# kav-institute/SemanticLiDARUnc

Hardware: AMD Instinct MI355X
Metric: range-image scans/sec (64x2048, T=8 MC) (higher is better)
Workload: dtype f16 (fp16 activations/weights, fp32 accumulate + epilogue, fp32 logits); 1 GPU; SalsaNext MC-dropout T=8 + entropy/MI map + IoU/ECE accumulation, 8 scans of 64x2048x5 per step per GPU (BASELINE configs[2] shape); T=8, parallelism=scan-sharded x1, mc_schedule=every pass fully recomputed

## Files before the change

semanticlidarunc_amd/csrc/conv_tail_h8.hip:

```cpp
#include "h8_common.h"

namespace {

struct TailArgs {
  const uint4 *a1, *a2;
  const uint4 *w2, *w1;
  const float *biasA, *bnA_a, *bnA_b, *biasB, *bnB_a, *bnB_b;
  float slopeA, slopeB;
  const uint2* resid;
  const uint4* sc_x;
  const uint4* sc_w;
  const float* sc_bias;
  float slopeS;
  uint2* out;
  int N, H, W, G;
  int tiles_x, tiles_y;
#ifdef SLU_H8_AB
  int dbg;
#endif
};

template <int MB, int WM, int WN, int RPW, bool W3RES>
__global__ __launch_bounds__(64 * WM * WN, 2) void tail_h8_kernel(const TailArgs a) {
  constexpr int NWAVE = WM * WN, T = 4, PAD = 1, DIL = 2;
// ... 441 lines not shown
              }
              const half8 bf = __builtin_bit_cast(half8, make_uint4(u[0], u[1], u[2], u[3]));
#pragma unroll
              for (int io = 0; io < MB; ++io) acco[io][b] = __builtin_amdgcn_mfma_f32_32x32x16_f16(wf[io], bf, acco[io][b], 0, 0, 0);
            }
          }
      }
    };
    h8_static_for(position, std::make_integer_sequence<int, NKS>{});
    first = false;

    if constexpr (HASRES) {
      asm volatile("s_waitcnt vmcnt(%8)"
                   : "+v"(res[0][0][0]), "+v"(res[0][0][1]), "+v"(res[(1 / NB) % MB][1 % NB][0]), "+v"(res[(1 / NB) % MB][1 % NB][1]),
                     "+v"(res[(2 / NB) % MB][2 % NB][0]), "+v"(res[(2 / NB) % MB][2 % NB][1]), "+v"(res[(3 / NB) % MB][3 % NB][0]), "+v"(res[(3 / NB) % MB][3 % NB][1])
                   : "n"(RESWAIT));
    }
    if constexpr (RES == 2) {
      static_assert(NKX * NB == 4, "the wait below names its registers");
      asm volatile("s_waitcnt vmcnt(%4)" : "+v"(xs[0][0]), "+v"(xs[0][NB - 1]), "+v"(xs[NKX - 1][0]), "+v"(xs[NKX - 1][NB - 1]) : "n"(RESWAIT));
    }
#pragma unroll
    for (int i = 0; i < MB; ++i)
#pragma unroll
      for (int b = 0; b < NB; ++b) {
        const int gy = cur.y0 + wn * RPW + (b >> 1), gx = cur.x0 + (b & 1) * 32 + jj;
        const bool ok = gy < a.H && gx < a.W;
        const size_t idx0 = ok ? ((size_t)cur.n * a.G + i * 4 + hh) * HW + (size_t)gy * a.W + gx : 0;
        f32x16 sacc;
        if constexpr (RES == 2) {
          sacc = f32x16{};
#pragma unroll
          for (int k = 0; k < NKX; ++k)
            sacc = __builtin_amdgcn_mfma_f32_32x32x16_f16(__builtin_bit_cast(half8, s_ws[(i * NKX + k) * 64 + lane]), __builtin_bit_cast(half8, xs[k][b]), sacc, 0, 0, 0);
        }
#pragma unroll
        for (int pr = 0; pr < 2; ++pr) {
          uint4 rw = make_uint4(0u, 0u, 0u, 0u);
          if constexpr (HASRES) rw = h8_swap16(res[i][b][pr].x, res[i][b][pr].y, res[i][b][pr].z, res[i][b][pr].w);
          unsigned hw[4];
#pragma unroll
          for (int q2 = 0; q2 < 2; ++q2) {
            const int q = 2 * pr + q2;
            const int c4 = (i * 32 + 8 * q) / 4;
            H8Quad t = h8_epilogue(acco[i][b], q, se4(3 * C / 4 + c4), se4(4 * C / 4 + c4), se4(5 * C / 4 + c4), slB);
            if constexpr (HASRES) h8_add_resid(t, q2 ? make_uint2(rw.z, rw.w) : make_uint2(rw.x, rw.y));
            if constexpr (RES == 2) {
              const H8Quad u = h8_bias_leaky(sacc, q, se4(6 * C / 4 + c4), slS);
              t.t0 += round_f16(u.t0);
              t.t1 += round_f16(u.t1);
            }
            hw[2 * q2] = pack2(t.t0);
            hw[2 * q2 + 1] = pack2(t.t1);
          }
          const uint4 rec = h8_swap16(hw[0], hw[1], hw[2], hw[3]);
          *(ok ? reinterpret_cast<uint4*>(a.out) + idx0 + (size_t)(2 * pr) * HW : &h8_trash_rec) = rec;
        }
      }
    asm volatile("" ::: "memory");
    cur = nxt;
    has_next = tile + 2 * t_step < t_end;
    if (has_next) nxt = decode(tile + 2 * t_step);
  }
  asm volatile("s_waitcnt vmcnt(0)" ::: "memory");
}

template <int MB, int RPW, int D, int RES>
int launch_tail2(TailArgs& a, const SluEmit& e) {
  constexpr int TH = 8 * RPW, C = 32 * MB, NKS = 2 * MB;
  constexpr size_t nblk_b = (size_t)(2 * (TH + 2) * 66 + 63) / 64;
  constexpr size_t lds = ((size_t)MB * NKS * 4 * 64 + (size_t)MB * 3 * NKS * 64 + (RES == 2 ? (size_t)MB * 2 * 64 : 0) + (size_t)D * nblk_b * 64 + 64) * 16;
  static_assert(lds + 7 * C * 4 <= 160 * 1024, "ring does not fit in LDS");
  a.tiles_x = (a.W + 63) / 64;
  a.tiles_y = (a.H + TH - 1) / TH;
  const long long nt = (long long)a.tiles_x * a.tiles_y * a.N;
  if (nt <= 0 || nt > 0x7fffffffLL) return SLU_EUNSUPPORTED;
  long long gx = 256;
  if (gx > nt) gx = nt;
  if (e.name) return slu_emit_name(e, "tail2_h8_kernel<%d, %d, %d, %d>", MB, RPW, D, RES);
  static SluLdsGrant grant;
  return slu_launch_lds(tail2_h8_kernel<MB, RPW, D, RES>, dim3((unsigned)gx), dim3(512), lds, e.st, grant, a);
}

template <int MB, int WM, int WN, int RPW, bool W3RES>
int launch_tail(TailArgs& a, const SluEmit& e) {
  constexpr int TH = WN * RPW, MBLK = MB * WM, C = 32 * MBLK, NKS = 2 * MBLK;
  constexpr size_t nb_alloc = (size_t)((2 * (TH + 2) * 66 + 63) / 64) * 64;
  constexpr size_t lds = (size_t)6 * C * 4 + 2 * nb_alloc * 16 + (size_t)2 * MBLK * 5 * 64 * 16 + (W3RES ? (size_t)MBLK * NKS * 64 * 16 : 0) +
                         (size_t)(C / 8) * TH * 64 * 16;
  static_assert(lds <= 160 * 1024, "tile does not fit in LDS");
  a.tiles_x = (a.W + 63) / 64;
  a.tiles_y = (a.H + TH - 1) / TH;
  const long long nt = (long long)a.tiles_x * a.tiles_y * a.N;
  if (nt <= 0 || nt > 0x7fffffffLL) return SLU_EUNSUPPORTED;
  long long gx = 256;
  if (gx > nt) gx = nt;
  if (e.name) return slu_emit_name(e, "tail_h8_kernel<%d, %d, %d, %d, %s>", MB, WM, WN, RPW, slu_tf(W3RES));
  static SluLdsGrant grant;
  return slu_launch_lds(tail_h8_kernel<MB, WM, WN, RPW, W3RES>, dim3((unsigned)gx), dim3(64 * WM * WN), lds, e.st, grant, a);
}

}

extern "C" int slu_conv_tail_h8_shortcut_supported(int C, int sc_cin) { return C == 64 && sc_cin == 32 ? 1 : 0; }

extern "C" int slu_conv_tail_h8_supported(int C, int H, int W) { return (C == 32 || C == 64 || C == 128) && H > 0 && W > 0 ? 1 : 0; }

static int conv_tail_dispatch(const slu_conv_tail_h8_desc* d, const SluEmit& e) {
  if (!d || !d->a1 || !d->a2 || !d->w2x2 || !d->w1x1 || !d->out || d->N <= 0 || d->H <= 0 || d->W <= 0) return SLU_EINVAL;
  if (((uintptr_t)d->a1 | (uintptr_t)d->a2 | (uintptr_t)d->out | (uintptr_t)d->resid | (uintptr_t)d->w2x2 | (uintptr_t)d->w1x1) & 15) return SLU_EINVAL;
  if ((d->bnA_a == nullptr) != (d->bnA_b == nullptr) || (d->bnB_a == nullptr) != (d->bnB_b == nullptr)) return SLU_EINVAL;
  if (!slu_conv_tail_h8_supported(d->C, d->H, d->W)) return SLU_EUNSUPPORTED;
  if (d->hasactA && !(d->slopeA >= 0.0f && d->slopeA <= 1.0f)) return SLU_EINVAL;
  if (d->hasactB && !(d->slopeB >= 0.0f && d->slopeB <= 1.0f)) return SLU_EINVAL;
  TailArgs a{};
  a.a1 = reinterpret_cast<const uint4*>(d->a1);
  a.a2 = reinterpret_cast<const uint4*>(d->a2);
  a.w2 = reinterpret_cast<const uint4*>(d->w2x2);
  a.w1 = reinterpret_cast<const uint4*>(d->w1x1);
  a.biasA = d->biasA; a.bnA_a = d->bnA_a; a.bnA_b = d->bnA_b;
  a.biasB = d->biasB; a.bnB_a = d->bnB_a; a.bnB_b = d->bnB_b;
  a.slopeA = d->hasactA ? d->slopeA : 1.0f;
  a.slopeB = d->hasactB ? d->slopeB : 1.0f;
  a.resid = reinterpret_cast<const uint2*>(d->resid);
  a.out = reinterpret_cast<uint2*>(d->out);
  a.N = d->N; a.H = d->H; a.W = d->W; a.G = d->C / 8;
#ifdef SLU_H8_AB
  static const int dbg = slu_env_int("SLU_TAIL_DBG", 0);
  a.dbg = dbg;
#endif
  static const bool v1 = slu_env_int("SLU_TAIL_V1", 0) == 1;
  if (d->sc_x) {
    if (d->resid || !d->sc_w || !slu_conv_tail_h8_shortcut_supported(d->C, d->sc_cin) || (((uintptr_t)d->sc_x | (uintptr_t)d->sc_w) & 15)) return SLU_EINVAL;
    if (d->sc_hasact && !(d->sc_slope >= 0.0f && d->sc_slope <= 1.0f)) return SLU_EINVAL;
    a.sc_x = reinterpret_cast<const uint4*>(d->sc_x);
    a.sc_w = reinterpret_cast<const uint4*>(d->sc_w);
    a.sc_bias = d->sc_bias;
    a.slopeS = d->sc_hasact ? d->sc_slope : 1.0f;
    return launch_tail2<2, 1, 4, 2>(a, e);
  }
  if (!v1 && d->C == 32) return a.resid ? launch_tail2<1, 2, 3, 1>(a, e) : launch_tail2<1, 2, 3, 0>(a, e);
  if (!v1 && d->C == 64) return a.resid ? launch_tail2<2, 1, 4, 1>(a, e) : launch_tail2<2, 1, 4, 0>(a, e);
  if (d->C == 32) return launch_tail<1, 1, 8, 2, true>(a, e);
  if (d->C == 64) return launch_tail<2, 1, 8, 1, true>(a, e);
  return launch_tail<2, 2, 4, 1, false>(a, e);
}

extern "C" int slu_conv_tail_h8_fwd(const slu_conv_tail_h8_desc* d, slu_stream_t stream) { return conv_tail_dispatch(d, SluEmit{slu_stream(stream), nullptr, 0}); }

extern "C" int slu_conv_tail_h8_kernel_name(const slu_conv_tail_h8_desc* d, char* buf, size_t n) {
  return buf ? conv_tail_dispatch(d, SluEmit{nullptr, buf, n}) : SLU_EINVAL;
}
```

semanticlidarunc_amd/h8.py:

```python
from __future__ import annotations


import ctypes as C
from typing import NamedTuple, Optional, Sequence

import torch

from . import _lib, ops
from ._lib import ConvH8Desc, check
from .ops import _ptr, _req, _stream


class H8Source(NamedTuple):
    tensor: torch.Tensor
    scale: Optional[torch.Tensor] = None
    nbatch: int = 0
    shuffle: bool = False


def shuffle_store_perm(channels: int, device=None) -> torch.Tensor:
    if channels % 32:
        raise RuntimeError(f"shuffle_store_perm: {channels} channels are not whole groups of 32")
    key = (int(channels), None if device is None else str(device))
    perm = _STORE_PERM.get(key)
# ... 94 lines not shown
    n = None if n_out is None else int(n_out)
    if n is not None and n <= 0:
        raise RuntimeError(f"conv2d_h8: n_out={n_out} is not a positive number of images")
    h = w = None
    gin = 0
    keep = []
    for i, s in enumerate(srcs):
        t = _req_h8(s.tensor, f"src[{i}]")
        sn, sg, sh, sw, _ = t.shape
        gstored = sg
        if s.shuffle:
            if i != 0 or sg % 8 or s.nbatch:
                raise RuntimeError("src[0] only may be read through PixelShuffle in place, with whole groups of 64 stored channels")
            sg, sh, sw = sg // 4, 2 * sh, 2 * sw
        if s.nbatch:
            if n is None or sn != s.nbatch or n % sn:
                raise RuntimeError(f"src[{i}]: a batch-broadcast source must follow a full-batch source (or n_out be given) and divide N")
            sn = n
        if n is None:
            n = sn
        if h is None:
            h, w = sh, sw
        if (sn, sh, sw) != (n, h, w):
            raise RuntimeError(f"src[{i}]: spatial/batch size {(sn, sh, sw)} != {(n, h, w)}")
        if s.scale is not None:
            _req(s.scale, f"src[{i}].scale")
            if tuple(s.scale.shape) != (n, 8 * gstored):
                raise RuntimeError(f"src[{i}].scale: expected {(n, 8 * gstored)}, got {tuple(s.scale.shape)}")
        d.src[i].ptr, d.src[i].scale, d.src[i].G, d.src[i].nbatch = t.data_ptr(), _ptr(s.scale), gstored, int(s.nbatch)
        d.src[i].shuffle = 1 if s.shuffle else 0
        gin += sg
        keep.append(t)
    if not 8 * (gin - 1) < cin <= 8 * gin:
        raise RuntimeError(f"conv2d_h8: cin={cin} does not match {gin} input blocks")
    _req(wpack, "wpack", torch.uint8)
    if wpack.numel() != lib.slu_packed_weight_bytes_h8(cout, cin, ksize):
        raise RuntimeError(f"wpack: {wpack.numel()} bytes does not match Cout={cout} Cin={cin} k={ksize} (h8)")
    for t, nme in ((bias, "bias"), (bn_a, "bn_a"), (bn_b, "bn_b")):
        if t is not None:
            _req(t, nme)
            if t.numel() != cout:
                raise RuntimeError(f"{nme}: expected {cout} elements, got {t.numel()}")
    if (bn_a is None) != (bn_b is None):
        raise RuntimeError("bn_a and bn_b must be given together")
    gout = (cout + 7) // 8
    if out_f32_nchw:
        if resid is not None:
            raise RuntimeError("conv2d_h8: no residual on the fp32 NCHW output form")
        out = torch.empty((n, cout, h, w), dtype=torch.float32, device=keep[0].device)
    else:
        out = torch.empty((n, gout, h, w, 8), dtype=torch.float16, device=keep[0].device)
    if resid is not None:
        _req_h8(resid, "resid")
        if tuple(resid.shape) != (n, gout, h, w, 8):
            raise RuntimeError(f"resid: expected {(n, gout, h, w, 8)}, got {tuple(resid.shape)}")
    d.nsrc = len(srcs)
    d.N, d.H, d.W, d.Cout = n, h, w, cout
    d.ksize, d.dil, d.pad = ksize, dil, pad
    d.wpack, d.bias = wpack.data_ptr(), _ptr(bias)
    d.has_act, d.slope = (0, 0.0) if slope is None else (1, float(slope))
    d.bn_a, d.bn_b, d.resid, d.out = _ptr(bn_a), _ptr(bn_b), _ptr(resid), out.data_ptr()
    d.out_f32_nchw = 1 if out_f32_nchw else 0
    d.act_after_resid = 1 if act_after_resid else 0
    if ops.TIMING is None:
        check(lib.slu_conv2d_h8_fwd(C.byref(d), _stream()), "slu_conv2d_h8_fwd")
        return out
    buf = C.create_string_buffer(96)
    check(lib.slu_conv2d_h8_kernel_name(C.byref(d), buf, 96), "slu_conv2d_h8_kernel_name")
    e0, e1 = torch.cuda.Event(enable_timing=True), torch.cuda.Event(enable_timing=True)
    e0.record()
    check(lib.slu_conv2d_h8_fwd(C.byref(d), _stream()), "slu_conv2d_h8_fwd")
    e1.record()
    flops = 2.0 * cin * cout * ksize * ksize * n * h * w
    nbytes = n * h * w * (2.0 * cin + (4.0 if out_f32_nchw else 2.0) * cout) + 2.0 * cout * cin * ksize * ksize
    ops.TIMING.append((buf.value.decode(), flops, nbytes, e0, e1, nbytes + (n * h * w * 2.0 * cout if resid is not None else 0.0)))
    ops.TIMING_TAGS.append(f"N{n} {cin}->{cout} k{ksize}d{dil} {h}x{w}")
    return out


def conv_tail_supported(channels: int, h: int, w: int) -> bool:
    return bool(_lib.load().slu_conv_tail_h8_supported(int(channels), int(h), int(w)))


def conv_tail_shortcut_supported(channels: int, cin: int) -> bool:
    return bool(_lib.load().slu_conv_tail_h8_shortcut_supported(int(channels), int(cin)))


def conv_tail_h8(a1: torch.Tensor, a2: torch.Tensor, w2x2: torch.Tensor, w1x1: torch.Tensor,
                 bias_a: Optional[torch.Tensor], slope_a: Optional[float], bn_a: Optional[tuple],
                 bias_b: Optional[torch.Tensor], slope_b: Optional[float], bn_b: Optional[tuple],
                 resid: Optional[torch.Tensor] = None, shortcut: Optional[tuple] = None) -> torch.Tensor:
    lib = _lib.load()
    _req_h8(a1, "a1")
    _req_h8(a2, "a2")
    if a1.shape != a2.shape:
        raise RuntimeError(f"conv_tail_h8: a1 {tuple(a1.shape)} != a2 {tuple(a2.shape)}")
    n, g, h, w, _ = a1.shape
    c = 8 * g
    if not conv_tail_supported(c, h, w):
        raise RuntimeError(f"conv_tail_h8: C={c} is not covered by the fused kernel (use two conv2d_h8 calls)")
    _req(w2x2, "w2x2", torch.uint8)
    _req(w1x1, "w1x1", torch.uint8)
    if w2x2.numel() != lib.slu_packed_weight_bytes_h8(c, c, 2) or w1x1.numel() != lib.slu_packed_weight_bytes_h8(c, 3 * c, 1):
        raise RuntimeError("conv_tail_h8: packed weight sizes do not match C")
    d = _lib.ConvTailH8Desc()
    for name, t in (("bias_a", bias_a), ("bias_b", bias_b)) + tuple((f"bn_{k}[{i}]", v) for k, pair in (("a", bn_a), ("b", bn_b)) if pair is not None
                                                                       for i, v in enumerate(pair)):
        if t is not None:
            _req(t, name)
            if t.numel() != c:
                raise RuntimeError(f"{name}: expected {c} elements, got {t.numel()}")
    if resid is not None:
        _req_h8(resid, "resid")
        if resid.shape != a1.shape:
            raise RuntimeError(f"resid: expected {tuple(a1.shape)}, got {tuple(resid.shape)}")
    if shortcut is not None:
        sx, sw, sb, sslope, scin = shortcut
        if resid is not None:
            raise RuntimeError("conv_tail_h8: resid and shortcut are exclusive")
        if not conv_tail_shortcut_supported(c, scin):
            raise RuntimeError(f"conv_tail_h8: shortcut {scin} -> {c} is not covered (run the 1x1 conv and pass resid)")
        _req_h8(sx, "shortcut.x")
        _req(sw, "shortcut.w", torch.uint8)
        if tuple(sx.shape) != (n, scin // 8, h, w, 8) or sw.numel() != lib.slu_packed_weight_bytes_h8(c, scin, 1):
            raise RuntimeError("conv_tail_h8: shortcut operand sizes do not match")
        if sb is not None:
            _req(sb, "shortcut.bias")
            if sb.numel() != c:
                raise RuntimeError(f"shortcut.bias: expected {c} elements, got {sb.numel()}")
    out = torch.empty_like(a1)
    d.a1, d.a2, d.N, d.H, d.W, d.C = a1.data_ptr(), a2.data_ptr(), n, h, w, c
    if shortcut is not None:
        d.sc_x, d.sc_w, d.sc_bias, d.sc_cin = sx.data_ptr(), sw.data_ptr(), _ptr(sb), int(scin)
        d.sc_hasact, d.sc_slope = (0, 0.0) if sslope is None else (1, float(sslope))
    d.w2x2, d.w1x1 = w2x2.data_ptr(), w1x1.data_ptr()
    d.biasA, d.bnA_a, d.bnA_b = _ptr(bias_a), _ptr(None if bn_a is None else bn_a[0]), _ptr(None if bn_a is None else bn_a[1])
    d.biasB, d.bnB_a, d.bnB_b = _ptr(bias_b), _ptr(None if bn_b is None else bn_b[0]), _ptr(None if bn_b is None else bn_b[1])
    d.hasactA, d.slopeA = (0, 0.0) if slope_a is None else (1, float(slope_a))
    d.hasactB, d.slopeB = (0, 0.0) if slope_b is None else (1, float(slope_b))
    d.resid, d.out = _ptr(resid), out.data_ptr()
    if ops.TIMING is None:
        check(lib.slu_conv_tail_h8_fwd(C.byref(d), _stream()), "slu_conv_tail_h8_fwd")
        return out
    buf = C.create_string_buffer(96)
    check(lib.slu_conv_tail_h8_kernel_name(C.byref(d), buf, 96), "slu_conv_tail_h8_kernel_name")
    e0, e1 = torch.cuda.Event(enable_timing=True), torch.cuda.Event(enable_timing=True)
    e0.record()
    check(lib.slu_conv_tail_h8_fwd(C.byref(d), _stream()), "slu_conv_tail_h8_fwd")
    e1.record()
    scin = shortcut[4] if shortcut is not None else 0
    flops = 2.0 * c * (c * (4 + 3) + scin) * n * h * w
    nbytes = n * h * w * 2.0 * (c + c + 3 * c + c + (scin + c if shortcut is not None else 0)) + 2.0 * c * (c * (4 + 3) + scin)
    min_bytes = n * h * w * 2.0 * (c * 3 + (c if resid is not None else 0) + scin) + 2.0 * c * (c * (4 + 3) + scin)
    ops.TIMING.append((buf.value.decode(), flops, nbytes, e0, e1, min_bytes))
    ops.TIMING_TAGS.append(f"N{n} {c}->{c} k2d2 + {3 * c}->{c} k1" + (f" + {scin}->{c} k1 shortcut" if shortcut is not None else "") + f" fused {h}x{w}")
    return out


def ctx_block_supported(cin: int, c: int, h: int, w: int) -> bool:
    return bool(_lib.load().slu_ctx_block_h8_supported(int(cin), int(c), int(h), int(w)))


def ctx_block_h8(x: torch.Tensor, cin: int, w1: torch.Tensor, w2: torch.Tensor, w3: torch.Tensor, bias1: Optional[torch.Tensor],
                 bias2: Optional[torch.Tensor], bn1: Optional[tuple], bias3: Optional[torch.Tensor], bn2: Optional[tuple],
                 slope: float, n_out: Optional[int] = None) -> torch.Tensor:
    lib = _lib.load()
    _req_h8(x, "x")
    nimg, g, h, w, _ = x.shape
    n = nimg if n_out is None else int(n_out)
    if n <= 0 or n % nimg:
        raise RuntimeError(f"ctx_block_h8: n_out={n} is not a multiple of the {nimg} input images")
    if not 8 * (g - 1) < cin <= 8 * g or not ctx_block_supported(cin, 32, h, w):
        raise RuntimeError(f"ctx_block_h8: cin={cin} with {g} input blocks is not covered by the fused kernel")
    for t, nme, shape in ((w1, "w1", (32, cin, 1)), (w2, "w2", (32, 32, 3)), (w3, "w3", (32, 32, 3))):
        _req(t, nme, torch.uint8)
        if t.numel() != lib.slu_packed_weight_bytes_h8(*shape):
            raise RuntimeError(f"{nme}: packed weight size does not match {shape}")
    vecs = (("bias1", bias1), ("bias2", bias2), ("bias3", bias3)) + tuple((f"bn{k}[{i}]", v) for k, pair in ((1, bn1), (2, bn2)) if pair is not None
                                                                           for i, v in enumerate(pair))
    for name, t in vecs:
        if t is not None:
            _req(t, name)
            if t.numel() != 32:
                raise RuntimeError(f"{name}: expected 32 elements, got {t.numel()}")
    out = torch.empty((n, 4, h, w, 8), dtype=torch.float16, device=x.device)
    d = _lib.CtxBlockH8Desc()
    d.x, d.N, d.H, d.W, d.Cin, d.C = x.data_ptr(), n, h, w, int(cin), 32
    d.w1, d.w2, d.w3 = w1.data_ptr(), w2.data_ptr(), w3.data_ptr()
    d.bias1, d.bias2, d.bias3 = _ptr(bias1), _ptr(bias2), _ptr(bias3)
    d.bn1_a, d.bn1_b = _ptr(None if bn1 is None else bn1[0]), _ptr(None if bn1 is None else bn1[1])
    d.bn2_a, d.bn2_b = _ptr(None if bn2 is None else bn2[0]), _ptr(None if bn2 is None else bn2[1])
    d.slope, d.out = float(slope), out.data_ptr()
    d.nbatch = 0 if n == nimg else nimg
    if ops.TIMING is None:
        check(lib.slu_ctx_block_h8_fwd(C.byref(d), _stream()), "slu_ctx_block_h8_fwd")
        return out
    e0, e1 = torch.cuda.Event(enable_timing=True), torch.cuda.Event(enable_timing=True)
    e0.record()
    check(lib.slu_ctx_block_h8_fwd(C.byref(d), _stream()), "slu_ctx_block_h8_fwd")
    e1.record()
    px = float(n * h * w)
    flops = 2.0 * (cin * 32 + 2 * 9 * 32 * 32) * px
    nbytes = px * 2.0 * ((8 * g + 32) + (32 + 32) + (32 + 32)) + 2.0 * (32 * cin + 2 * 9 * 32 * 32)
    min_bytes = float(h * w) * 2.0 * (nimg * 8 * g + n * 32) + 2.0 * (32 * cin + 2 * 9 * 32 * 32)
    ops.TIMING.append((f"ctx_h8_kernel<{1 if cin <= 16 else 2}>", flops, nbytes, e0, e1, min_bytes))
    ops.TIMING_TAGS.append(f"N{n} {cin}->32 k1 + 32->32 k3d1 + 32->32 k3d2 fused {h}x{w}")
    return out


def head_mc_h8(x: torch.Tensor, wpack: torch.Tensor, bias: Optional[torch.Tensor], classes: int, passes: int, batch: int, eps: float = 1e-12):
    _req_h8(x, "x")
    n, g, h, w, _ = x.shape
    if n != passes * batch:
# ... 214 lines not shown
```

semanticlidarunc_amd/salsanext.py:

```python
from __future__ import annotations

import os
from typing import Dict, Optional

import torch
import torch.nn as nn

from . import autograd as _autograd
from . import h8, ops
from .autograd import AvgPoolFn, ConvLayerFn, LayerCfg
from .ops import ConvSource

_SLOPE = 0.01

CONV_PRECISIONS = ("fp32", "f16x3", "f16")
_CONV_PRECISION = os.environ.get("SLU_CONV_PRECISION", "fp32")
_TRAIN_CONV_PRECISION = os.environ.get("SLU_TRAIN_CONV_PRECISION", "fp32")
_FUSE_TAIL = os.environ.get("SLU_FUSE_TAIL", "1") != "0"
_FUSE_TAIL_MAX_C = int(os.environ.get("SLU_FUSE_TAIL_MAX_C", "64"))
_FUSE_SHORTCUT = os.environ.get("SLU_FUSE_SHORTCUT", "1") != "0"
_FUSE_CTX = os.environ.get("SLU_FUSE_CTX", "1") != "0"
_PACK_MULTI = os.environ.get("SLU_PACK_MULTI", "1") != "0"
_FUSE_HEAD_MC = os.environ.get("SLU_FUSE_HEAD_MC", "1") != "0"
_MC_BCAST_INPUT = os.environ.get("SLU_MC_BCAST_INPUT", "1") != "0"
# ... 11 lines not shown
def set_conv_precision(precision: str) -> None:
    global _CONV_PRECISION
    if precision not in CONV_PRECISIONS:
        raise ValueError(f"unknown conv precision {precision!r}; choose from {CONV_PRECISIONS}")
    _CONV_PRECISION = precision


def get_conv_precision() -> str:
    return _CONV_PRECISION


class _Prepared:

    __slots__ = ("key", "wpack", "bn_key", "bn_a", "bn_b", "dgrad", "key16", "wpack16", "key8", "wpack8", "key8p", "wpack8p", "vecp_key", "vecp")

    def __init__(self):
        self.key = self.bn_key = None
        self.key8p = self.wpack8p = self.vecp_key = self.vecp = None
        self.wpack = self.bn_a = self.bn_b = None
        self.key16 = self.wpack16 = None
        self.key8 = self.wpack8 = None
        self.dgrad = {}


def _tkey(*ts):
    return tuple((t.data_ptr(), t._version, t.device) for t in ts)


class _FusedBlock(nn.Module):

    def __call__(self, *args, **kwargs):
        _autograd.nbt_scope_enter()
        try:
            return super().__call__(*args, **kwargs)
        finally:
            _autograd.nbt_scope_exit()

    def _folded_bn(self, p: _Prepared, bn: Optional[nn.BatchNorm2d]):
        if bn is None:
            return None, None
        bkey = _tkey(bn.weight, bn.bias, bn.running_mean, bn.running_var)
        if p.bn_key != bkey:
            p.bn_a, p.bn_b = ops.bn_fold(bn.weight.detach(), bn.bias.detach(), bn.running_mean, bn.running_var, bn.eps)
            p.bn_key = bkey
        return p.bn_a, p.bn_b

    def _permuted_h8(self, p: _Prepared, conv: nn.Conv2d, bn):
        wkey = _tkey(conv.weight)
        if p.key8p != wkey:
            perm = h8.shuffle_store_perm(conv.out_channels, conv.weight.device)
            p.wpack8p = h8.pack_conv_weight_h8(conv.weight.detach().index_select(0, perm).contiguous())
            p.key8p = wkey
        bn_a, bn_b = self._folded_bn(p, bn)
        vkey = (p.bn_key if bn is not None else None, None if conv.bias is None else _tkey(conv.bias))
        if p.vecp_key != vkey:
            perm = h8.shuffle_store_perm(conv.out_channels, conv.weight.device)
            p.vecp = tuple(None if v is None else v.detach().index_select(0, perm).contiguous() for v in (conv.bias, bn_a, bn_b))
            p.vecp_key = vkey
        return (p.wpack8p,) + p.vecp

    def _run_h8(self, p: _Prepared, conv: nn.Conv2d, bn, srcs, resid, act, out_f32, out_perm=False):
        if out_perm:
            wpack, bias, bn_a, bn_b = self._permuted_h8(p, conv, bn)
        else:
            wkey = _tkey(conv.weight)
            if p.key8 != wkey:
                p.wpack8 = h8.pack_conv_weight_h8(conv.weight.detach().contiguous())
                p.key8 = wkey
            wpack, bias = p.wpack8, None if conv.bias is None else conv.bias.detach()
            bn_a, bn_b = self._folded_bn(p, bn)
        return h8.conv2d_h8([h8.H8Source(s.tensor, s.scale, s.nbatch, bool(s.pixel_shuffle)) for s in srcs], wpack,
                            conv.in_channels, conv.out_channels, conv.kernel_size[0], conv.dilation[0], conv.padding[0],
                            bias=bias, slope=_SLOPE if act else None, bn_a=bn_a, bn_b=bn_b, resid=resid, out_f32_nchw=out_f32)

    def _prepared(self, conv: nn.Conv2d) -> _Prepared:
        cache: Dict[str, _Prepared] = self.__dict__.setdefault("_prep", {})
        p = cache.get(str(id(conv)))
        if p is None:
            p = cache[str(id(conv))] = _Prepared()
        return p

    def _tail_is_fused(self, conv_a: nn.Conv2d, conv_b: nn.Conv2d, a1) -> bool:
        c = conv_a.out_channels
        return bool(_FUSE_TAIL and a1.dtype == torch.float16 and a1.dim() == 5 and conv_a.kernel_size == (2, 2) and conv_a.dilation == (2, 2)
                    and conv_b.kernel_size == (1, 1) and conv_b.in_channels == 3 * c and conv_b.out_channels == c
                    and c <= _FUSE_TAIL_MAX_C and h8.conv_tail_supported(c, a1.shape[2], a1.shape[3]))

    def _run_tail(self, conv_a: nn.Conv2d, bn_a, conv_b: nn.Conv2d, bn_b, a1, a2, resid=None, shortcut=None, out_perm=False):
        if out_perm and a1.dtype != torch.float16:
            raise RuntimeError("a block output in shuffle order exists on the half-precision inference path only")
        if out_perm and shortcut is not None and self._tail_is_fused(conv_a, conv_b, a1):
            raise RuntimeError("a block output in shuffle order: the shortcut computed inside the fused tail is not permuted")
        if self._tail_is_fused(conv_a, conv_b, a1):
            packs, folded, biases = [], [], []
            for conv, bn, perm in ((conv_a, bn_a, False), (conv_b, bn_b, out_perm)):
                p = self._prepared(conv)
                if perm:
                    wp, bias, fa, fb = self._permuted_h8(p, conv, bn)
                    packs.append(wp)
                    biases.append(bias)
                    folded.append(None if fa is None else (fa, fb))
                    continue
                wkey = _tkey(conv.weight)
                if p.key8 != wkey:
                    p.wpack8 = h8.pack_conv_weight_h8(conv.weight.detach().contiguous())
                    p.key8 = wkey
                packs.append(p.wpack8)
                biases.append(None if conv.bias is None else conv.bias.detach())
                fa, fb = self._folded_bn(p, bn)
                folded.append(None if fa is None else (fa, fb))
            sc = None
            if shortcut is not None:
                sx, sconv = shortcut
                p = self._prepared(sconv)
                wkey = _tkey(sconv.weight)
                if p.key8 != wkey:
                    p.wpack8 = h8.pack_conv_weight_h8(sconv.weight.detach().contiguous())
                    p.key8 = wkey
                sc = (sx, p.wpack8, None if sconv.bias is None else sconv.bias.detach(), _SLOPE, sconv.in_channels)
            return h8.conv_tail_h8(a1, a2, packs[0], packs[1], biases[0], _SLOPE, folded[0], biases[1], _SLOPE, folded[1], resid=resid, shortcut=sc)
        if shortcut is not None:
            resid = self._run(shortcut[1], None, [ConvSource(shortcut[0])], out_perm=out_perm)
        a3 = self._run(conv_a, bn_a, [ConvSource(a2)])
        return self._run(conv_b, bn_b, [ConvSource(a1), ConvSource(a2), ConvSource(a3)], resid=resid, out_perm=out_perm)

    def _run(self, conv: nn.Conv2d, bn: Optional[nn.BatchNorm2d], srcs, resid=None, act=True, out_f32=False, out_perm=False):
        cache: Dict[str, _Prepared] = self.__dict__.setdefault("_prep", {})
        name = str(id(conv))
        p = cache.get(name)
        if p is None:
            p = cache[name] = _Prepared()
        if srcs[0].tensor.dtype == torch.float16:
            return self._run_h8(p, conv, bn, srcs, resid, act, out_f32, out_perm)
        if out_perm:
            raise RuntimeError("an output in shuffle order exists on the half-precision inference path only")
        wkey = _tkey(conv.weight)
        if p.key != wkey:
            p.wpack = ops.pack_conv_weight(conv.weight.detach().contiguous())
            p.key = wkey
        k = conv.kernel_size[0]
        slope = _SLOPE if act else None
        wants_grad = torch.is_grad_enabled() and (
            conv.weight.requires_grad or any(s.tensor.requires_grad for s in srcs)
            or (resid is not None and resid.requires_grad) or (bn is not None and bn.weight.requires_grad))
        if wants_grad or (bn is not None and bn.training):
            wp = p.wpack
            if _TRAIN_CONV_PRECISION == "f16x3":
                if p.key16 != wkey:
                    p.wpack16 = ops.pack_conv_weight_f16x3(conv.weight.detach().contiguous())
                    p.key16 = wkey
                wp = p.wpack16
            cfg = LayerCfg(k, conv.dilation[0], conv.padding[0], slope, [s.scale for s in srcs],
                           [s.pixel_shuffle for s in srcs], bn, conv.out_channels, wp, p.dgrad, _TRAIN_CONV_PRECISION)
            return ConvLayerFn.apply(cfg, conv.weight, conv.bias, None if bn is None else bn.weight,
                                     None if bn is None else bn.bias, resid, *[s.tensor for s in srcs])
        bn_a, bn_b = self._folded_bn(p, bn)
        wpack, precision = p.wpack, "fp32"
        if _CONV_PRECISION == "f16x3":
            precision = "f16x3"
            if p.key16 != wkey:
                p.wpack16 = ops.pack_conv_weight_f16x3(conv.weight.detach().contiguous())
                p.key16 = wkey
            wpack = p.wpack16
        return ops.conv2d_fused(srcs, wpack, conv.out_channels, k, conv.dilation[0], conv.padding[0],
                                bias=None if conv.bias is None else conv.bias.detach(),
                                slope=slope, bn_a=bn_a, bn_b=bn_b, resid=resid, precision=precision)


_DROPOUT_KERNEL = os.environ.get("SLU_DROPOUT_KERNEL", "1") != "0"
# ... 411 lines not shown
```

Baseline: 747.9 scans/s.

## Add fused 128-channel conv tail kernel with staged weight ring and register-streamed inputs

Adds a dedicated fused tail kernel for 128-channel blocks. It computes the dilated 2x2 conv and keeps its output image in LDS, then runs the 1x1 conv over the concatenated three inputs, streaming the a1/a2 groups through registers. The Python side now enables tail fusion above the 64-channel cap whenever the dispatcher picks this kernel, which it does when there are at least 256 tiles. This should remove the separate unfused conv launches and the intermediate tensor traffic for the deepest blocks. In exchange it adds hand-counted vmcnt waits that are fragile, and the emitted kernel name is reused to tell Python the fusion is available.

Measured after the change: 766.9 scans/s (median of 6 runs). +2.5%, better.

```diff
diff --git a/semanticlidarunc_amd/csrc/conv_tail128_h8.h b/semanticlidarunc_amd/csrc/conv_tail128_h8.h
--- /dev/null
+++ b/semanticlidarunc_amd/csrc/conv_tail128_h8.h
@@ -0,0 +1,283 @@
+
+template <bool HASRES>
+__device__ __forceinline__ void tail128_h8_body(const TailArgs& a) {
+  constexpr int NWAVE = 8, WN = 4, MBW = 2, RPW = 2, T = 4, PAD = 1, DIL = 2, D = 3;
+  constexpr int C = 128, NKS = 8, MBLK = 4;
+  constexpr int TW = 64, TH = WN * RPW, NB = 2 * RPW;
+  constexpr int LW = TW + 2 * PAD, LH = TH + 2 * PAD, REC = LH * LW;
+  constexpr int NBLK_B = (2 * REC + 63) / 64, NBLK_A = MBLK * T, NBLK = NBLK_B + NBLK_A;
+  constexpr int NIB = (NBLK + NWAVE - 1) / NWAVE;
+  constexpr int SLOTREC = NBLK * 64;
+  constexpr int IMGREC = (C / 8) * TH * 64;
+  constexpr int NPAIR = 3 * NKS / 2, NRG = NKS;
+  constexpr int WPREC = 2 * MBLK * 64;
+  static_assert(D * SLOTREC <= IMGREC, "the phase-A ring lives inside the a3 image");
+  static_assert(NBLK_B == 21 && NIB == 5 && NB == 4 && MBW * NB == 8, "the counted waits below name their registers and counts");
+  constexpr int W_A = NIB;
+  constexpr int W_A7 = 2;
+  constexpr int W_B0 = 8;
+  constexpr int W_BR = 9;
+  constexpr int W_B7 = 1;
+  constexpr int W_B8 = 1;
+  constexpr int W_B9 = 9;
+  constexpr int W_B10 = 9;
+  constexpr int W_B11 = 8;
+  constexpr int W_XA = 8, W_XB = 8;
+
+  __shared__ __attribute__((aligned(16))) float s_epi[6 * C];
+  extern __shared__ __attribute__((aligned(16))) char smem[];
+  uint4* s_a3 = reinterpret_cast<uint4*>(smem);
+  uint4* s_wb = s_a3 + IMGREC;
+  uint4* s_trash = s_wb + 3 * WPREC;
+
+  const int tid = threadIdx.x, lane = tid & 63, wave = __builtin_amdgcn_readfirstlane(tid >> 6), wm = wave >> 2, wn = wave & 3;
+  const int hh = lane >> 5, jj = lane & 31;
+  const size_t HW = (size_t)a.H * a.W;
+
+  const H8Run run = h8_tile_run(a.tiles_x, a.tiles_y, a.N);
+  const int t_beg = run.beg, t_end = run.end, t_step = run.step;
+  if (t_beg >= t_end) return;
+
+  if (tid < C) {
+    H8_FILL_EPI(s_epi, 0, C, tid, true, tid, a.biasA, a.bnA_a, a.bnA_b);
+    H8_FILL_EPI(s_epi, 3 * C, C, tid, true, tid, a.biasB, a.bnB_a, a.bnB_b);
+  }
+
+  struct TilePos { int x0, y0, n; };
+  auto decode = [&](int t) {
+    TilePos p;
+    const int tx = t % a.tiles_x;
+    t /= a.tiles_x;
+    p.x0 = tx * TW;
+    p.y0 = (t % a.tiles_y) * TH;
+    p.n = t / a.tiles_y;
+    return p;
+  };
+  H8_OPAQUE_ADDR(zero, h8_zero_rec);
+  H8_OPAQUE_ADDR(trash, h8_trash_rec);
+  auto lane_again = [&]() {
+    int l = lane;
+    asm volatile("" : "+v"(l));
+    return l;
+  };
+  auto stage = [&](const TilePos& tp, int c, int slot) {
+    uint4* db = s_a3 + slot * SLOTREC;
+    const uintptr_t base0 = reinterpret_cast<uintptr_t>(a.a2) +
+                            16 * ((long long)(((size_t)tp.n * a.G + 2 * c) * HW) + (long long)(tp.y0 - PAD) * a.W + (tp.x0 - PAD));
+    const int l = lane_again();
+#pragma unroll
+    for (int i = 0; i < NIB; ++i) {
+      const int blk = i * NWAVE + wave;
+      uintptr_t p = zero;
+      if (i * NWAVE < NBLK_B) {
+        const int e = blk * 64 + l;
+        const int g2 = e / REC, rem = e - g2 * REC, r = rem / LW, cc = rem - r * LW;
+        const int gy = tp.y0 - PAD + r, gx = tp.x0 - PAD + cc;
+        const bool ok = e < 2 * REC && (unsigned)gy < (unsigned)a.H && (unsigned)gx < (unsigned)a.W;
+        const long long off = (long long)(g2 ? HW : 0) + r * a.W + cc;
+        p = ok ? base0 + 16 * off : zero;
+      }
+      if ((i + 1) * NWAVE > NBLK_B && blk >= NBLK_B) {
+        const int ab = blk - NBLK_B, m = ab >> 2, tap = ab & 3;
+        uintptr_t wsrc = reinterpret_cast<uintptr_t>(a.w2 + (((size_t)m * NKS + c) * T + tap) * 64);
+        asm volatile("" : "+s"(wsrc));
+        p = blk < NBLK ? wsrc + 16 * l : zero;
+      }
+      SLU_GLDS16(reinterpret_cast<const uint4*>(p), blk < NBLK ? db + blk * 64 : s_trash);
+    }
+    asm volatile("" ::: "memory");
+  };
+  auto stage_w = [&](int j) {
+    uintptr_t wsrc = reinterpret_cast<uintptr_t>(a.w1 + ((size_t)(wave & 3) * 3 * NKS + 2 * j + (wave >> 2)) * 64);
+    asm volatile("" : "+s"(wsrc));
+    const uintptr_t p = wsrc + 16 * lane_again();
+    SLU_GLDS16(reinterpret_cast<const uint4*>(p), s_wb + (j % 3) * WPREC + wave * 64);
+    asm volatile("" ::: "memory");
+  };
+
+  const int bbase2 = hh * REC + (wn * RPW) * LW + jj;
+  const float2v slA = {a.slopeA, a.slopeA}, slB = {a.slopeB, a.slopeB};
+  int se_i = hh + wm * MBW * 8, s3_i = ((((wm * MBW * 4) * TH + wn * RPW) * 64 + jj) << 1) + hh;
+  int a3_lo = (hh * TH + wn * RPW) * 64 + jj, a3_hi = a3_lo + IMGREC / 2;
+  asm volatile("" : "+v"(se_i), "+v"(a3_lo), "+v"(a3_hi));
+  const unsigned s3_addr = (unsigned)(uintptr_t)((__attribute__((address_space(3))) char*)smem) + s3_i * 8;
+  auto se4 = [&](int k) { return reinterpret_cast<const f32x4v*>(s_epi)[se_i + k]; };
+  __syncthreads();
+
+  for (int tile = t_beg; tile < t_end; tile += t_step) {
+    const TilePos cur = decode(tile);
+    f32x16 acc[MBW][NB];
+    u32x4v rg[2][2][NB];
+    u32x4v res[HASRES ? MBW : 1][HASRES ? NB : 1][2];
+    h8_zero(acc);
+    unsigned voff[NB];
+    bool okb[NB];
+#pragma unroll
+    for (int b = 0; b < NB; ++b) {
+      const int gy = cur.y0 + wn * RPW + (b >> 1), gx = cur.x0 + (b & 1) * 32 + jj;
+      okb[b] = gy < a.H && gx < a.W;
+      voff[b] = (unsigned)(((okb[b] ? (size_t)gy * a.W + gx : 0) + hh * HW) << 4);
+    }
+    const unsigned long long img16 = 16ull * ((size_t)cur.n * a.G * HW);
+    auto load_group = [&](auto jc) {
+      constexpr int j = decltype(jc)::value;
+      auto& dst = rg[j & 1];
+      const unsigned long long base = reinterpret_cast<unsigned long long>(j < NRG / 2 ? a.a1 : a.a2) + img16;
+#pragma unroll
+      for (int kk = 0; kk < 2; ++kk)
+#pragma unroll
+        for (int b = 0; b < NB; ++b) {
+          const unsigned vo = voff[b];
+          const unsigned long long sb = base + 32ull * ((2 * j + kk) % NKS) * HW;
+          asm volatile("global_load_dwordx4 %0, %1, %2" : "=&v"(dst[kk][b]) : "v"(vo), "s"(sb) : "memory");
+        }
+    };
+    auto load_resid = [&](auto ic) {
+      constexpr int i = decltype(ic)::value;
+      if constexpr (HASRES) {
+        auto& dst = res[i];
+        const unsigned long long base = reinterpret_cast<unsigned long long>(a.resid) + img16;
+#pragma unroll
+        for (int b = 0; b < NB; ++b)
+#pragma unroll
+          for (int pr = 0; pr < 2; ++pr) {
+            const unsigned vo = voff[b];
+            const unsigned long long sb = base + 16ull * ((wm * MBW + i) * 4 + 2 * pr) * HW;
+            asm volatile("global_load_dwordx4 %0, %1, %2" : "=&v"(dst[b][pr]) : "v"(vo), "s"(sb) : "memory");
+          }
+      }
+    };
+
+    h8_lds_barrier();
+    stage(cur, 0, 0);
+    stage(cur, 1, 1);
+    auto position_a = [&](auto cc) {
+      constexpr int c = decltype(cc)::value;
+      h8_vmcnt<(c < NKS - 1 ? W_A : W_A7)>();
+      h8_lds_barrier();
+      if constexpr (c + 2 < NKS) stage(cur, c + 2, (c + 2) % D);
+      if constexpr (c == NKS - 2) { stage_w(0); stage_w(1); }
+      const uint4* sb = s_a3 + (c % D) * SLOTREC + bbase2;
+      const uint4* sa = s_a3 + (c % D) * SLOTREC + (NBLK_B + wm * MBW * T) * 64 + lane;
+      half8 fa[2][MBW], fb[2][NB];
+      auto rd = [&](int st, int buf) {
+        const int dy = (st >> 1) * DIL, dx = (st & 1) * DIL;
+#pragma unroll
+        for (int i = 0; i < MBW; ++i) fa[buf][i] = __builtin_bit_cast(half8, sa[(i * T + st) * 64]);
+#pragma unroll
+        for (int b = 0; b < NB; ++b) fb[buf][b] = __builtin_bit_cast(half8, sb[((b >> 1) + dy) * LW + (b & 1) * 32 + dx]);
+      };
+      rd(0, 0);
+#pragma unroll
+      for (int st = 0; st < T; ++st) {
+        if (st + 1 < T) rd(st + 1, (st + 1) & 1);
+        __builtin_amdgcn_sched_barrier(0);
+#pragma unroll
+        for (int b = 0; b < NB; ++b)
+#pragma unroll
+          for (int i = 0; i < MBW; ++i) acc[i][b] = __builtin_amdgcn_mfma_f32_32x32x16_f16(fa[st & 1][i], fb[st & 1][b], acc[i][b], 0, 0, 0);
+        __builtin_amdgcn_sched_barrier(0);
+      }
+      if constexpr (c == NKS - 1) {
+        load_group(std::integral_constant<int, 0>{});
+        load_group(std::integral_constant<int, 1>{});
+      }
+    };
+    h8_static_for(position_a, std::make_integer_sequence<int, NKS>{});
+
+    h8_lds_barrier();
+#pragma unroll
+    for (int i = 0; i < MBW; ++i)
+#pragma unroll
+      for (int b = 0; b < NB; ++b)
+#pragma unroll
+        for (int q = 0; q < 4; ++q) {
+          const int c4 = (i * 32 + 8 * q) / 4;
+          const uint2 v = pack4(h8_epilogue(acc[i][b], q, se4(c4), se4(C / 4 + c4), se4(2 * C / 4 + c4), slA));
+          const unsigned long long v64 = (unsigned long long)v.x | ((unsigned long long)v.y << 32);
+          asm volatile("ds_write_b64 %0, %1 offset:%2" ::"v"(s3_addr), "v"(v64), "n"(((((i * 4 + q) * TH + (b >> 1)) * 64 + (b & 1) * 32) << 1) * 8) : "memory");
+        }
+    h8_zero(acc);
+
+    auto position_b = [&](auto jc) {
+      constexpr int j = decltype(jc)::value;
+      constexpr int XA = HASRES ? 8 : 0;
+      if constexpr (j < NRG) {
+        constexpr int n = j == 0 ? W_B0 : (j == NRG - 1 ? W_B7 : W_BR);
+        asm volatile("s_waitcnt vmcnt(%8)"
+                     : "+v"(rg[j & 1][0][0]), "+v"(rg[j & 1][0][1]), "+v"(rg[j & 1][0][2]), "+v"(rg[j & 1][0][3]),
+                       "+v"(rg[j & 1][1][0]), "+v"(rg[j & 1][1][1]), "+v"(rg[j & 1][1][2]), "+v"(rg[j & 1][1][3])
+                     : "n"(n)
+                     : "memory");
+      } else {
+        h8_vmcnt<(j == 8 ? W_B8 : j == 9 ? W_B9 - 8 + XA : j == 10 ? W_B10 - 8 + XA : W_B11 - 8 + XA)>();
+      }
+      h8_lds_barrier();
+      if constexpr (j + 2 < NPAIR) stage_w(j + 2);
+      if constexpr (j == 8) load_resid(std::integral_constant<int, 0>{});
+      if constexpr (j == 10) load_resid(std::integral_constant<int, 1>{});
+      const uint4* sw = s_wb + (j % 3) * WPREC + (wm * MBW) * 64 + lane;
+#pragma unroll
+      for (int kk = 0; kk < 2; ++kk) {
+        half8 af[MBW], bf[NB];
+#pragma unroll
+        for (int i = 0; i < MBW; ++i) af[i] = __builtin_bit_cast(half8, sw[(kk * MBLK + i) * 64]);
+#pragma unroll
+        for (int b = 0; b < NB; ++b) {
+          if constexpr (j < NRG) bf[b] = __builtin_bit_cast(half8, rg[j & 1][kk][b]);
+          else bf[b] = __builtin_bit_cast(half8, s_a3[(j < NRG + 2 ? a3_lo : a3_hi) + ((2 * ((2 * (j - NRG) + kk) & 3)) * TH + (b >> 1)) * 64 + (b & 1) * 32]);
+        }
+#pragma unroll
+        for (int b = 0; b < NB; ++b)
+#pragma unroll
+          for (int i = 0; i < MBW; ++i) acc[i][b] = __builtin_amdgcn_mfma_f32_32x32x16_f16(af[i], bf[b], acc[i][b], 0, 0, 0);
+        if constexpr (j >= NRG) __builtin_amdgcn_sched_barrier(0);
+      }
+      if constexpr (j + 2 < NRG) {
+        __builtin_amdgcn_sched_barrier(0);
+        load_group(std::integral_constant<int, j + 2>{});
+      }
+    };
+    h8_static_for(position_b, std::make_integer_sequence<int, NPAIR>{});
+
+    auto epilogue_b = [&](auto ic) {
+      constexpr int i = decltype(ic)::value;
+      if constexpr (HASRES) {
+        asm volatile("s_waitcnt vmcnt(%8)"
+                     : "+v"(res[i][0][0]), "+v"(res[i][0][1]), "+v"(res[i][1][0]), "+v"(res[i][1][1]),
+                       "+v"(res[i][2][0]), "+v"(res[i][2][1]), "+v"(res[i][3][0]), "+v"(res[i][3][1])
+                     : "n"(i == 0 ? W_XA : W_XB)
+                     : "memory");
+      }
+#pragma unroll
+      for (int b = 0; b < NB; ++b) {
+#pragma unroll
+        for (int pr = 0; pr < 2; ++pr) {
+          uint4 rw = make_uint4(0u, 0u, 0u, 0u);
+          if constexpr (HASRES) rw = h8_swap16(res[i][b][pr].x, res[i][b][pr].y, res[i][b][pr].z, res[i][b][pr].w);
+          unsigned hw[4];
+#pragma unroll
+          for (int q2 = 0; q2 < 2; ++q2) {
+            const int q = 2 * pr + q2;
+            const int c4 = (i * 32 + 8 * q) / 4;
+            H8Quad t = h8_epilogue(acc[i][b], q, se4(3 * C / 4 + c4), se4(4 * C / 4 + c4), se4(5 * C / 4 + c4), slB);
+            if constexpr (HASRES) h8_add_resid(t, q2 ? make_uint2(rw.z, rw.w) : make_uint2(rw.x, rw.y));
+            hw[2 * q2] = pack2(t.t0);
+            hw[2 * q2 + 1] = pack2(t.t1);
+          }
+          const uint4 rec = h8_swap16(hw[0], hw[1], hw[2], hw[3]);
+          const uintptr_t dst = reinterpret_cast<uintptr_t>(a.out) + img16 + 16ull * ((wm * MBW + i) * 4 + 2 * pr) * HW;
+          *reinterpret_cast<__attribute__((address_space(1))) u32x4v*>(okb[b] ? dst + voff[b] : trash) = u32x4v{rec.x, rec.y, rec.z, rec.w};
+        }
+      }
+      asm volatile("" ::: "memory");
+    };
+    h8_static_for(epilogue_b, std::make_integer_sequence<int, MBW>{});
+  }
+}
+
+template <bool HASRES>
+__global__ __launch_bounds__(512, 2) void tail128_h8_kernel(const TailArgs a) { tail128_h8_body<HASRES>(a); }
+
+inline bool tail128_fits(int G, int H, int W) { return (unsigned long long)G * H * W * 16ull < (1ull << 32); }
+constexpr size_t tail128_lds_bytes() { return ((size_t)16 * 8 * 64 + 3 * 2 * 4 * 64 + 64) * 16; }
diff --git a/semanticlidarunc_amd/csrc/conv_tail_h8.hip b/semanticlidarunc_amd/csrc/conv_tail_h8.hip
--- a/semanticlidarunc_amd/csrc/conv_tail_h8.hip
+++ b/semanticlidarunc_amd/csrc/conv_tail_h8.hip
@@ -547,6 +547,24 @@
   return slu_launch_lds(tail2_h8_kernel<MB, RPW, D, RES>, dim3((unsigned)gx), dim3(512), lds, e.st, grant, a);
 }
 
+#include "conv_tail128_h8.h"
+
+inline long long tail128_tiles(int N, int H, int W) { return (long long)((W + 63) / 64) * ((H + 7) / 8) * N; }
+
+template <int RES>
+int launch_tail128(TailArgs& a, const SluEmit& e) {
+  static_assert(tail128_lds_bytes() + 6 * 128 * 4 <= 160 * 1024, "image and weight ring do not fit in LDS");
+  a.tiles_x = (a.W + 63) / 64;
+  a.tiles_y = (a.H + 7) / 8;
+  const long long nt = tail128_tiles(a.N, a.H, a.W);
+  if (nt <= 0 || nt > 0x7fffffffLL) return SLU_EUNSUPPORTED;
+  long long gx = 256;
+  if (gx > nt) gx = nt;
+  if (e.name) return slu_emit_name(e, "tail2_h8_kernel<%d, %d, %d, %d>", 4, 2, 3, RES);
+  static SluLdsGrant grant;
+  return slu_launch_lds(tail128_h8_kernel<RES == 1>, dim3((unsigned)gx), dim3(512), tail128_lds_bytes(), e.st, grant, a);
+}
+
 template <int MB, int WM, int WN, int RPW, bool W3RES>
 int launch_tail(TailArgs& a, const SluEmit& e) {
   constexpr int TH = WN * RPW, MBLK = MB * WM, C = 32 * MBLK, NKS = 2 * MBLK;
@@ -570,6 +588,11 @@
 extern "C" int slu_conv_tail_h8_shortcut_supported(int C, int sc_cin) { return C == 64 && sc_cin == 32 ? 1 : 0; }
 
 extern "C" int slu_conv_tail_h8_supported(int C, int H, int W) { return (C == 32 || C == 64 || C == 128) && H > 0 && W > 0 ? 1 : 0; }
+
+static bool tail128_chosen(int C, int N, int H, int W) {
+  static const int min_tiles = slu_env_int("SLU_TAIL128_MIN_TILES", 256);
+  return C == 128 && N > 0 && H > 0 && W > 0 && tail128_tiles(N, H, W) >= (min_tiles > 256 ? min_tiles : 256) && tail128_fits(C / 8, H, W);
+}
 
 static int conv_tail_dispatch(const slu_conv_tail_h8_desc* d, const SluEmit& e) {
   if (!d || !d->a1 || !d->a2 || !d->w2x2 || !d->w1x1 || !d->out || d->N <= 0 || d->H <= 0 || d->W <= 0) return SLU_EINVAL;
@@ -606,6 +629,7 @@
   }
   if (!v1 && d->C == 32) return a.resid ? launch_tail2<1, 2, 3, 1>(a, e) : launch_tail2<1, 2, 3, 0>(a, e);
   if (!v1 && d->C == 64) return a.resid ? launch_tail2<2, 1, 4, 1>(a, e) : launch_tail2<2, 1, 4, 0>(a, e);
+  if (!v1 && tail128_chosen(d->C, d->N, d->H, d->W)) return a.resid ? launch_tail128<1>(a, e) : launch_tail128<0>(a, e);
   if (d->C == 32) return launch_tail<1, 1, 8, 2, true>(a, e);
   if (d->C == 64) return launch_tail<2, 1, 8, 1, true>(a, e);
   return launch_tail<2, 2, 4, 1, false>(a, e);
diff --git a/semanticlidarunc_amd/h8.py b/semanticlidarunc_amd/h8.py
--- a/semanticlidarunc_amd/h8.py
+++ b/semanticlidarunc_amd/h8.py
@@ -200,6 +200,23 @@
     return bool(_lib.load().slu_conv_tail_h8_supported(int(channels), int(h), int(w)))
 
 
+_TAIL_NAMES: dict = {}
+
+
+def conv_tail_kernel_name(channels: int, n: int, h: int, w: int, resid: bool) -> str:
+    key = (int(channels), int(n), int(h), int(w), bool(resid))
+    name = _TAIL_NAMES.get(key)
+    if name is None:
+        d = _lib.ConvTailH8Desc()
+        d.a1 = d.a2 = d.w2x2 = d.w1x1 = d.out = 0x1000
+        d.resid = 0x1000 if resid else None
+        d.C, d.N, d.H, d.W = key[:4]
+        buf = C.create_string_buffer(96)
+        check(_lib.load().slu_conv_tail_h8_kernel_name(C.byref(d), buf, 96), "slu_conv_tail_h8_kernel_name")
+        name = _TAIL_NAMES[key] = buf.value.decode()
+    return name
+
+
 def conv_tail_shortcut_supported(channels: int, cin: int) -> bool:
     return bool(_lib.load().slu_conv_tail_h8_shortcut_supported(int(channels), int(cin)))
 
@@ -207,7 +224,7 @@
 def conv_tail_h8(a1: torch.Tensor, a2: torch.Tensor, w2x2: torch.Tensor, w1x1: torch.Tensor,
                  bias_a: Optional[torch.Tensor], slope_a: Optional[float], bn_a: Optional[tuple],
                  bias_b: Optional[torch.Tensor], slope_b: Optional[float], bn_b: Optional[tuple],
-                 resid: Optional[torch.Tensor] = None, shortcut: Optional[tuple] = None) -> torch.Tensor:
+                 resid: Optional[torch.Tensor] = None, shortcut: Optional[tuple] = None, out: Optional[torch.Tensor] = None) -> torch.Tensor:
     lib = _lib.load()
     _req_h8(a1, "a1")
     _req_h8(a2, "a2")
@@ -246,7 +263,12 @@
             _req(sb, "shortcut.bias")
             if sb.numel() != c:
                 raise RuntimeError(f"shortcut.bias: expected {c} elements, got {sb.numel()}")
-    out = torch.empty_like(a1)
+    if out is None:
+        out = torch.empty_like(a1)
+    else:
+        _req_h8(out, "out")
+        if out.shape != a1.shape:
+            raise RuntimeError(f"out: expected {tuple(a1.shape)}, got {tuple(out.shape)}")
     d.a1, d.a2, d.N, d.H, d.W, d.C = a1.data_ptr(), a2.data_ptr(), n, h, w, c
     if shortcut is not None:
         d.sc_x, d.sc_w, d.sc_bias, d.sc_cin = sx.data_ptr(), sw.data_ptr(), _ptr(sb), int(scin)
diff --git a/semanticlidarunc_amd/salsanext.py b/semanticlidarunc_amd/salsanext.py
--- a/semanticlidarunc_amd/salsanext.py
+++ b/semanticlidarunc_amd/salsanext.py
@@ -117,9 +117,11 @@
 
     def _tail_is_fused(self, conv_a: nn.Conv2d, conv_b: nn.Conv2d, a1) -> bool:
         c = conv_a.out_channels
-        return bool(_FUSE_TAIL and a1.dtype == torch.float16 and a1.dim() == 5 and conv_a.kernel_size == (2, 2) and conv_a.dilation == (2, 2)
-                    and conv_b.kernel_size == (1, 1) and conv_b.in_channels == 3 * c and conv_b.out_channels == c
-                    and c <= _FUSE_TAIL_MAX_C and h8.conv_tail_supported(c, a1.shape[2], a1.shape[3]))
+        if not (_FUSE_TAIL and a1.dtype == torch.float16 and a1.dim() == 5 and conv_a.kernel_size == (2, 2) and conv_a.dilation == (2, 2)
+                and conv_b.kernel_size == (1, 1) and conv_b.in_channels == 3 * c and conv_b.out_channels == c
+                and h8.conv_tail_supported(c, a1.shape[2], a1.shape[3])):
+            return False
+        return c <= _FUSE_TAIL_MAX_C or h8.conv_tail_kernel_name(c, a1.shape[0], a1.shape[2], a1.shape[3], False).startswith("tail2_h8_kernel<")
 
     def _run_tail(self, conv_a: nn.Conv2d, bn_a, conv_b: nn.Conv2d, bn_b, a1, a2, resid=None, shortcut=None, out_perm=False):
         if out_perm and a1.dtype != torch.float16:
```
